# Bluear7878/Remote-Sensing-Vision-Language-Diffusion-Model

Hardware: AMD Instinct MI355X
Metric: 512px x8 SR images/sec @50 steps (higher is better)
Workload: dtype f16 / bf16 MFMA operands as hi + lo pairs and triples, f32 accumulation and f32 residual streams (Stage 1: f16 tensors x f16 weight pairs; Stage 2: rsvld_amd.ops.UNET_POLICY; config.precision) -- the composition inside 1e-3 of the reference's CPU path (config.tolerance)

## Files before the change

include/rsvld_hip.h:

```cpp
#ifndef RSVLD_HIP_H
#define RSVLD_HIP_H

#include <stdint.h>

#ifdef __cplusplus
extern "C" {
#endif

#define RSVLD_OK 0
#define RSVLD_EINVAL (-1)
#define RSVLD_EUNSUPPORTED (-2)
#define RSVLD_ELAUNCH (-3)

#define RSVLD_F16 0
#define RSVLD_BF16 1
#define RSVLD_F32 2
#define RSVLD_SPLIT 3
#define RSVLD_F16W2 4
#define RSVLD_F16Q8 6
#define RSVLD_F16W1 5

#define RSVLD_ACT_NONE 0
#define RSVLD_ACT_SILU 1
#define RSVLD_ACT_GEGLU 2

const char* rsvld_version(void);

typedef struct rsvld_conv_desc {
    const void* x;
    const void* x2;
    const void* w;
    const float* bias;
    const float* rowvec;
    const void* residual;
    void* out;
    int32_t B, H, W, Cin, Cin2, Cout;
    int32_t KH, KW, stride, pad_t, pad_l, Ho, Wo;
    int32_t upsample;
    int32_t dtype;
    int32_t out_f32;
    int32_t act;
    float alpha, beta;
    int32_t rowvec_stride;
    int32_t plan_div;
    int32_t tune;
} rsvld_conv_desc;

#define RSVLD_TUNE_TILE_MASK 7
#define RSVLD_TUNE_STAGES_SHIFT 3
#define RSVLD_TUNE_NO_KSPLIT (1 << 6)
#define RSVLD_TUNE_REG_STAGING (1 << 7)
#define RSVLD_TUNE_HALO_NW4 (1 << 8)
#define RSVLD_TUNE_HALO_NW8 (1 << 9)
#define RSVLD_TUNE_NO_GEMM256 (1 << 10)
#define RSVLD_TUNE_GEMM_ONE_TILE (1 << 12)
#define RSVLD_TUNE_F32_SPLIT (1 << 11)

#define RSVLD_HQ8_SX_LO 14
#define RSVLD_HQ8_SX_HI 2
#define RSVLD_HQ8_SW_HI 6
#define RSVLD_HQ8_SW_LO 18
int rsvld_conv2d_nhwc(const rsvld_conv_desc* d, void* stream);

int rsvld_conv3x3_halo_supported(const rsvld_conv_desc* d);
int rsvld_conv3x3_halo_nhwc(const rsvld_conv_desc* d, const float* norm_scale_shift, int norm_silu,
                            float* out_stats_partials, void* stream);

int64_t rsvld_groupnorm_ws_bytes(int B, int HW, int C, int groups);
int rsvld_groupnorm_nhwc(const void* x, const void* x2, void* y,
                         const float* gamma, const float* beta,
                         const void* mod_scale1p, const void* mod_shift, int mod_stride,
                         int B, int HW, int C1, int C2, int groups, float eps,
                         int silu, int dtype, void* ws, void* stream);
int rsvld_groupnorm_stats(const void* x, const void* x2, float* mean_var,
                          int B, int HW, int C1, int C2, int groups,
                          int dtype, void* ws, void* stream);
int rsvld_groupnorm_apply(const void* x, const void* x2, void* y, const float* mean_var,
                          const float* gamma, const float* beta,
                          const void* mod_scale1p, const void* mod_shift, int mod_stride,
                          int B, int HW, int C1, int C2, int groups, float eps,
                          int silu, int dtype, void* stream);

int rsvld_groupnorm_scale_shift(const void* x, const void* x2, const float* gamma, const float* beta,
                                float* scale_shift, int B, int HW, int C1, int C2, int groups, float eps,
                                int dtype, void* ws, void* stream);

int rsvld_groupnorm_scale_shift_from_partials(const float* part1, int ntiles1, int C1,
                                              const float* part2, int ntiles2, int C2,
                                              const float* gamma, const float* beta, float* scale_shift,
                                              int B, int HW, int groups, float eps, void* stream);

int rsvld_layernorm(const void* x, void* y, const float* gamma, const float* beta,
                    int64_t rows, int C, float eps, int dtype, void* stream);

int rsvld_attention(const void* q, const void* k, const void* v, void* out,
                    int B, int heads, int Nq, int Nk, int D,
                    int64_t q_batch_stride, int64_t q_tok_stride,
                    int64_t k_batch_stride, int64_t k_tok_stride,
                    int64_t v_batch_stride, int64_t v_tok_stride,
                    int64_t o_batch_stride, int64_t o_tok_stride,
                    float scale, int dtype, int plan_div, void* ws, void* stream);
#define RSVLD_ATTN_D64_FOUR_WAVE 1
#define RSVLD_ATTN_D64_PINGPONG 2
#define RSVLD_ATTN_D64_PIPELINED 3
int rsvld_attention_tuned(const void* q, const void* k, const void* v, void* out,
                          int B, int heads, int Nq, int Nk, int D,
                          int64_t q_batch_stride, int64_t q_tok_stride,
                          int64_t k_batch_stride, int64_t k_tok_stride,
                          int64_t v_batch_stride, int64_t v_tok_stride,
                          int64_t o_batch_stride, int64_t o_tok_stride,
                          float scale, int dtype, int plan_div, void* ws, void* stream, int tune);
int64_t rsvld_attention_ws_bytes(int B, int heads, int Nq, int Nk, int D, int plan_div);

int rsvld_linear_small_f32(const float* x, const float* w, const float* b, float* y,
                           int rows, int in_f, int out_f, int act_in, int act_out, void* stream);

int rsvld_sinusoidal_embedding(const float* t, float* out, int rows, int dim, int kind, void* stream);

int rsvld_nchw_f32_to_nhwc(const float* src, void* dst, int B, int C, int H, int W,
                           int Cdst, int c_off, int zero_pad, float scale, int dtype, void* stream);
int rsvld_nhwc_to_nchw_f32(const void* src, float* dst, int B, int C, int H, int W,
                           int Csrc, int c_off, int src_f32, int dtype, void* stream);
int rsvld_axpby(const void* a, const void* b, void* out, int64_t n, float sa, float sb,
                int dtype, void* stream);
int rsvld_geglu(const void* in, void* out, int64_t rows, int C, int dtype, void* stream);

int rsvld_ddpm_step(const float* x, const float* eps_nhwc, const float* noise, float* x_out,
                    int B, int C, int H, int W, int eps_c,
                    float c_recip, float c_recipm1, float coef1, float coef2, float sigma,
                    int clip, void* stream);

int rsvld_denoiser_out(const float* net_out_nhwc, const float* input, float* out,
                       int B, int C, int H, int W, int c_pad, float c_out, float c_skip, void* stream);
int rsvld_lerp_f32(const float* a, const float* b, float* out, int64_t n, float w, void* stream);
int rsvld_axpy_f32(const float* x, const float* y, float* out, int64_t n, float s, void* stream);
int rsvld_euler_step(const float* x_hat, const float* denoised, const float* x_center, float* x_out,
                     int64_t n, float restore_w, float sigma_hat, float dt, void* stream);
int rsvld_tile_blend_accumulate(float* acc, float* cnt, const float* tile, const float* weights,
                                int B, int C, int H, int W, int y0, int x0, int th, int tw, void* stream);
int rsvld_tile_blend_finish(const float* acc, const float* cnt, float* out, int64_t n, void* stream);
int64_t rsvld_absdiff_ws_bytes(int rows, int64_t n_per_row);
int rsvld_absdiff_sums(const void* a, const void* b, float* out, int rows, int64_t n_per_row,
                       int dtype, void* ws, void* stream);

int rsvld_gaussian_sample(const void* moments_nhwc, const float* noise, float* z,
                          int B, int C, int H, int W, int m_c, float scale, int src_f32,
                          int dtype, void* stream);

int rsvld_wavelet_blur(const float* img, float* low, float* high_accum, int planes, int H, int W,
                       int radius, void* stream);
int rsvld_add_f32(const float* a, const float* b, float* out, int64_t n, void* stream);
int rsvld_adain(const float* content, const float* style, float* out, float* ws_stats,
                int planes, int64_t HW, void* stream);

int rsvld_concat_c(const void* a, const void* b, void* out, int64_t rows, int C1, int C2,
                   int dtype, void* stream);

int rsvld_conv2d_nhwc_f32(const rsvld_conv_desc* d, void* stream);
int64_t rsvld_groupnorm_f32_ws_bytes(int B, int HW, int C, int groups);
int rsvld_groupnorm_stats_f32(const float* x, float* mean_var, int B, int HW, int C, int groups, void* ws, void* stream);
int rsvld_groupnorm_apply_f32(const float* x, float* y, const float* mean_var, const float* gamma, const float* beta,
                              const float* mod_scale1p, const float* mod_shift, int mod_stride,
                              int B, int HW, int C, int groups, float eps, int silu, void* stream);
int rsvld_attention_f32(const float* q, const float* k, const float* v, float* out,
                        int B, int heads, int Nq, int Nk, int D,
                        int64_t q_batch_stride, int64_t q_tok_stride,
                        int64_t k_batch_stride, int64_t k_tok_stride,
                        int64_t v_batch_stride, int64_t v_tok_stride,
                        int64_t o_batch_stride, int64_t o_tok_stride,
                        float scale, void* stream);
int rsvld_attention_f32_split(const float* q, const float* k, const float* v, float* out,
                              int B, int heads, int Nq, int Nk, int D,
                              int64_t q_batch_stride, int64_t q_tok_stride,
                              int64_t k_batch_stride, int64_t k_tok_stride,
                              int64_t v_batch_stride, int64_t v_tok_stride,
                              int64_t o_batch_stride, int64_t o_tok_stride,
                              float scale, void* stream);
int rsvld_layernorm_f32(const float* x, float* y, const float* gamma, const float* beta, int64_t rows, int C, float eps,
                        void* stream);
int rsvld_concat_c_f32(const float* a, const float* b, float* out, int64_t rows, int C1, int C2, void* stream);
int rsvld_axpby_f32(const float* a, const float* b, float* out, int64_t n, float sa, float sb, void* stream);
int rsvld_absdiff_sums_f32(const float* a, const float* b, float* out, int rows, int64_t n_per_row, void* stream);
int rsvld_nchw_f32_to_nhwc_f32(const float* src, float* dst, int B, int C, int H, int W,
                               int Cdst, int c_off, int zero_pad, float scale, void* stream);

int rsvld_gemv(const void* w, const void* x, const void* bias, void* y, int N, int K, int dtype, void* stream);
int rsvld_gemv_fused(const void* w, const void* x, const void* bias, const void* norm_w, float norm_eps, const void* residual, int glu,
// ... 44 lines not shown
```

remote-sensing-vision-language-diffusion-model_amd/csrc/attention.hip:

```cpp
#include "rsvld_common.h"
#include <type_traits>
#include <utility>

namespace {

struct AttnArgs {
    const void* q;
    const void* k;
    const void* v;
    void* out;
    int B, heads, Nq, Nk, D;
    int64_t q_bs, q_ts, k_bs, k_ts, v_bs, v_ts, o_bs, o_ts;
    float scale_log2e;
    unsigned long long* dbg;
};

typedef const __attribute__((address_space(1))) void* gptr_t;
typedef __attribute__((address_space(3))) void* lptr_t;

template <typename F, int... I> __device__ __forceinline__ void static_for_impl(F&& f, std::integer_sequence<int, I...>) {
    (f(std::integral_constant<int, I>{}), ...);
}
template <int N, typename F> __device__ __forceinline__ void static_for(F&& f) {
    static_for_impl(f, std::make_integer_sequence<int, N>{});
// ... 253 lines not shown
#define S_NXT snext
#define A5B_STEADY 0
#define dma_kb_s dma_kb
#define dma_k_s dma_k
#define dma_v_s dma_v
#include "attention_d512_body.inc"
#undef dma_kb_s
#undef dma_k_s
#undef dma_v_s
#undef A5B_STEADY
#undef S_CUR
#undef S_NXT
#undef A5B_PAIR
    }
#undef A5B_NOHOOK
#undef A5B_MFMA_NAME
#undef A5B_CHAIN
#undef A5B_STEP4
#if A5B_FINE
#undef A5B_STEPH4
#undef A5B_STEPH
#endif
#undef A5B_STEP
#undef A5B_KREAD

    const float l_tot = l_run + __shfl_xor(l_run, 32);
    if (qrow >= p.Nq) return;
    const float inv = 1.0f / l_tot;
    if (nsplit == 1) {
        T* Ob = (T*)p.out + (int64_t)b * p.o_bs + (int64_t)h * D + (int64_t)qrow * p.o_ts;
#pragma unroll
        for (int dt = 0; dt < 16; ++dt)
#pragma unroll
            for (int g = 0; g < 4; ++g) {
                v4 o;
#pragma unroll
                for (int e = 0; e < 4; ++e) o[e] = (T)(oacc[dt][4 * g + e] * inv);
                *(v4*)(Ob + dt * 32 + 8 * g + 4 * lh) = o;
            }
    } else {
        const int64_t row = ((int64_t)split * gridDim.z + blockIdx.z) * p.Nq + qrow;
        float* Po = part_o + row * D;
#pragma unroll
        for (int dt = 0; dt < 16; ++dt)
#pragma unroll
            for (int g = 0; g < 4; ++g) {
                f32x4 o;
#pragma unroll
                for (int e = 0; e < 4; ++e) o[e] = oacc[dt][4 * g + e] * inv;
                *(f32x4*)(Po + dt * 32 + 8 * g + 4 * lh) = o;
            }
        if (lh == 0) {
            part_ml[row * 2] = m_run;
            part_ml[row * 2 + 1] = l_tot;
        }
    }
}

template <typename T>
__global__ __launch_bounds__(128) void attn_combine_kernel(AttnArgs p, int nsplit, const float* part_o, const float* part_ml) {
    constexpr int D = 512;
    typedef typename Mfma<T>::v4 v4;
    const int qrow = blockIdx.x, bh = blockIdx.y;
    const int b = bh / p.heads, h = bh % p.heads;
    const int64_t nrows = (int64_t)gridDim.y * p.Nq;
    float mmax = -INFINITY;
    for (int i = 0; i < nsplit; ++i) mmax = fmaxf(mmax, part_ml[((int64_t)i * nrows + (int64_t)bh * p.Nq + qrow) * 2]);
    float wsum = 0.f;
    f32x4 acc = {0.f, 0.f, 0.f, 0.f};
    for (int i = 0; i < nsplit; ++i) {
        const int64_t row = (int64_t)i * nrows + (int64_t)bh * p.Nq + qrow;
        const float wi = part_ml[row * 2 + 1] * __builtin_amdgcn_exp2f(part_ml[row * 2] - mmax);
        const f32x4 o = *(const f32x4*)(part_o + row * D + threadIdx.x * 4);
        acc += o * wi;
        wsum += wi;
    }
    const float inv = 1.0f / wsum;
    v4 o;
#pragma unroll
    for (int e = 0; e < 4; ++e) o[e] = (T)(acc[e] * inv);
    *(v4*)((T*)p.out + (int64_t)b * p.o_bs + (int64_t)h * D + (int64_t)qrow * p.o_ts + threadIdx.x * 4) = o;
}

}

namespace {

constexpr int A6B_TILE = 64 * 128;
#ifndef A6B_ABL
#define A6B_ABL 0
#endif
#ifndef A6B_SUMCHK
#define A6B_SUMCHK 1
#endif
#ifndef A6B_KPB8
#define A6B_KPB8 1
#endif
#ifndef A6B_NW16_MIN
#define A6B_NW16_MIN (1 << 30)
#endif
#ifndef A6B_STAMP
#define A6B_STAMP 0
#endif
__device__ __forceinline__ unsigned long long a6b_stamp() {
    unsigned long long t;
    __builtin_amdgcn_sched_barrier(0);
    asm volatile("s_memtime %0\n\ts_waitcnt lgkmcnt(0)" : "=s"(t) :: "memory");
    __builtin_amdgcn_sched_barrier(0);
    return t;
}

#ifndef A6B_OCC4
#define A6B_OCC4 1
#endif
#ifndef A6B_BIAS
#define A6B_BIAS 1
#endif
__device__ __forceinline__ float a6b_add(float a, float b) { return a + b; }

#ifndef A6_STAGE_O
#define A6_STAGE_O 1
#endif
template <typename T>
__device__ __forceinline__ void a6_store_o(char* wbuf, const f32x16 (&oacc)[2], float inv, int q0, int lane, const AttnArgs& p, int b, int h) {
    typedef typename Mfma<T>::v4 v4;
    const int l31 = lane & 31, lh = lane >> 5;
    T* Ob = (T*)p.out + (int64_t)b * p.o_bs + (int64_t)h * 64;
    if (!A6_STAGE_O) {
        if (q0 + l31 >= p.Nq) return;
#pragma unroll
        for (int dt = 0; dt < 2; ++dt)
#pragma unroll
            for (int g = 0; g < 4; ++g) {
                v4 o;
#pragma unroll
                for (int e = 0; e < 4; ++e) o[e] = (T)(oacc[dt][4 * g + e] * inv);
                *(v4*)(Ob + (int64_t)(q0 + l31) * p.o_ts + dt * 32 + 8 * g + 4 * lh) = o;
            }
        return;
    }
#pragma unroll
    for (int dt = 0; dt < 2; ++dt)
#pragma unroll
        for (int g = 0; g < 4; ++g) {
            v4 o;
#pragma unroll
            for (int e = 0; e < 4; ++e) o[e] = (T)(oacc[dt][4 * g + e] * inv);
            *(v4*)(wbuf + l31 * 128 + (((dt * 4 + g) ^ (l31 & 7)) << 4) + lh * 8) = o;
        }
#pragma unroll
    for (int j = 0; j < 4; ++j) {
        const int row = (lane >> 3) + 8 * j, chunk = lane & 7;
        const u32x4 v = *(const u32x4*)(wbuf + row * 128 + ((chunk ^ (row & 7)) << 4));
        if (q0 + row < p.Nq) *(u32x4*)(Ob + (int64_t)(q0 + row) * p.o_ts + chunk * 8) = v;
    }
}

#ifndef A6B_NW8_MIN
#define A6B_NW8_MIN 16384
#endif
template <typename T, int NW>
__global__ __launch_bounds__(64 * NW, A6B_OCC4 ? 4 : 2) void attn_d64b_kernel(AttnArgs p) {
    constexpr int D = 64;
    constexpr int KPB = NW == 8 ? A6B_KPB8 : 1;
    constexpr int NB = 2 * KPB;
    constexpr bool SPLIT = NW == 16;
// ... 373 lines not shown
        return;
    }
    if (qrow >= p.Nq) return;
    T* Ob = (T*)p.out + (int64_t)b * p.o_bs + (int64_t)h * D + (int64_t)qrow * p.o_ts;
#pragma unroll
    for (int dt = 0; dt < 2; ++dt)
#pragma unroll
        for (int g = 0; g < 4; ++g) {
            v4 o;
#pragma unroll
            for (int e = 0; e < 4; ++e) o[e] = (T)(oacc[dt][4 * g + e] * inv);
            *(v4*)(Ob + dt * 32 + 8 * g + 4 * lh) = o;
        }
}

#include "attention_d64c.inc"
#include "attention_d64p.inc"

}

#ifndef A5B_MALL_KEYS
#define A5B_MALL_KEYS 65536
#endif
static void attn512_plan(int B, int heads, int Nq, int Nk, int* nsplit, int* keys_per_split) {
    const int64_t base = (int64_t)((Nq + 127) / 128) * B * heads;
    int ns = 1;
    if (base < 192) {
        ns = (int)((256 + base - 1) / base);
        const int cap = Nk / 256 > 1 ? Nk / 256 : 1;
        if (ns > cap) ns = cap;
        if (ns > 16) ns = 16;
    }
    if (A5B_MALL_KEYS > 0 && Nk > A5B_MALL_KEYS + A5B_MALL_KEYS / 2) {
        const int nm = (Nk + A5B_MALL_KEYS - 1) / A5B_MALL_KEYS;
        if (nm > ns) ns = nm;
    }
    int kps = ((Nk + ns - 1) / ns + 31) / 32 * 32;
    *keys_per_split = kps;
    *nsplit = (Nk + kps - 1) / kps;
}

extern "C" int64_t rsvld_attention_ws_bytes(int B, int heads, int Nq, int Nk, int D, int plan_div) {
    if (D != 512 || B <= 0 || heads <= 0 || Nq <= 0 || Nk <= 0) return 0;
    int ns, kps;
    attn512_plan(plan_div > 1 ? (B + plan_div - 1) / plan_div : B, heads, Nq, Nk, &ns, &kps);
    if (ns == 1) return 0;
    return (int64_t)ns * B * heads * Nq * (512 + 2) * 4;
}

extern "C" int rsvld_attention_tuned(const void* q, const void* k, const void* v, void* out, int B, int heads, int Nq, int Nk,
                                     int D, int64_t q_batch_stride, int64_t q_tok_stride, int64_t k_batch_stride,
                                     int64_t k_tok_stride, int64_t v_batch_stride, int64_t v_tok_stride,
                                     int64_t o_batch_stride, int64_t o_tok_stride, float scale, int dtype, int plan_div,
                                     void* ws, void* stream, int tune) {
    if (!q || !k || !v || !out || B <= 0 || heads <= 0 || Nq <= 0 || Nk <= 0) return RSVLD_EINVAL;
    if (dtype != RSVLD_F16 && dtype != RSVLD_BF16) return RSVLD_EINVAL;
    if ((q_tok_stride | k_tok_stride | v_tok_stride | o_tok_stride | q_batch_stride | k_batch_stride | v_batch_stride |
         o_batch_stride) & 7)
        return RSVLD_EINVAL;
    if (heads > 65535 || B > 65535) return RSVLD_EINVAL;
    AttnArgs a;
    a.q = q; a.k = k; a.v = v; a.out = out;
    a.B = B; a.heads = heads; a.Nq = Nq; a.Nk = Nk; a.D = D;
    a.q_bs = q_batch_stride; a.q_ts = q_tok_stride; a.k_bs = k_batch_stride; a.k_ts = k_tok_stride;
    a.v_bs = v_batch_stride; a.v_ts = v_tok_stride; a.o_bs = o_batch_stride; a.o_ts = o_tok_stride;
    a.scale_log2e = scale * 1.4426950408889634f;
    a.dbg = (A6B_STAMP && D == 64) ? (unsigned long long*)ws : nullptr;
    hipStream_t s = (hipStream_t)stream;
    if (D == 512) {
        int ns, kps;
        attn512_plan(plan_div > 1 ? (B + plan_div - 1) / plan_div : B, heads, Nq, Nk, &ns, &kps);
        if (ns > 1 && ws == nullptr) return RSVLD_EINVAL;
        float* part_o = (float*)ws;
        float* part_ml = ns > 1 ? part_o + (int64_t)ns * B * heads * Nq * 512 : nullptr;
        dim3 grid((unsigned)((Nq + 127) / 128), (unsigned)ns, (unsigned)(B * heads));
        const bool shared = k == v && k_batch_stride == v_batch_stride && k_tok_stride == v_tok_stride;
        auto go = [&](auto kern, auto comb, int smem) -> int {
            static const hipError_t attr = hipFuncSetAttribute((const void*)kern, hipFuncAttributeMaxDynamicSharedMemorySize, smem);
            if (attr != hipSuccess) return RSVLD_ELAUNCH;
            hipLaunchKernelGGL(kern, grid, dim3(256), smem, s, a, kps, part_o, part_ml);
            if (ns > 1) hipLaunchKernelGGL(comb, dim3((unsigned)Nq, (unsigned)(B * heads)), dim3(128), 0, s, a, ns, part_o, part_ml);
            return rsvld_check_launch();
        };
        if (shared)
            return dtype == RSVLD_F16 ? go(attn_d512b_kernel<f16, true>, attn_combine_kernel<f16>, A5B_SMEM_SH)
                                      : go(attn_d512b_kernel<bf16, true>, attn_combine_kernel<bf16>, A5B_SMEM_SH);
        return dtype == RSVLD_F16 ? go(attn_d512b_kernel<f16, false>, attn_combine_kernel<f16>, A5B_SMEM)
                                  : go(attn_d512b_kernel<bf16, false>, attn_combine_kernel<bf16>, A5B_SMEM);
    }
    if (D == 64) {
        const char force = tune == RSVLD_ATTN_D64_FOUR_WAVE ? 'b' : tune == RSVLD_ATTN_D64_PINGPONG ? 'c' : tune == RSVLD_ATTN_D64_PIPELINED ? 'p' : 0;
        if (force == 'p' && Nk > 64 && k_tok_stride < (1 << 23) && v_tok_stride < (1 << 23)) {
            dim3 grid((unsigned)((Nq + 255) / 256), (unsigned)heads, (unsigned)B);
            static const hipError_t a16 = hipFuncSetAttribute((const void*)attn_d64p_kernel<f16>, hipFuncAttributeMaxDynamicSharedMemorySize, A6P_SMEM);
            static const hipError_t abf = hipFuncSetAttribute((const void*)attn_d64p_kernel<bf16>, hipFuncAttributeMaxDynamicSharedMemorySize, A6P_SMEM);
            if (a16 != hipSuccess || abf != hipSuccess) return RSVLD_ELAUNCH;
            if (dtype == RSVLD_F16) hipLaunchKernelGGL((attn_d64p_kernel<f16>), grid, dim3(512), A6P_SMEM, s, a);
            else hipLaunchKernelGGL((attn_d64p_kernel<bf16>), grid, dim3(512), A6P_SMEM, s, a);
            return rsvld_check_launch();
        }
        const int64_t wg_c = (int64_t)((Nq + 511) / 512) * heads * B;
        const bool c_strides_ok = 64 * k_tok_stride * 2 < ((int64_t)1 << 32) && 64 * v_tok_stride * 2 < ((int64_t)1 << 32);
        if (force == 'c' && !c_strides_ok) return RSVLD_EUNSUPPORTED;
        if (c_strides_ok && (a.dbg == nullptr || force == 'c') && force != 'b' && Nk > 64 && ((wg_c >= A6C_MIN_WG && Nk >= A6C_MIN_KEYS) || force == 'c')) {
            dim3 grid((unsigned)((Nq + 511) / 512), (unsigned)heads, (unsigned)B);
            static const hipError_t attr16 = hipFuncSetAttribute((const void*)attn_d64c_kernel<f16>, hipFuncAttributeMaxDynamicSharedMemorySize, A6C_SMEM);
            static const hipError_t attrbf = hipFuncSetAttribute((const void*)attn_d64c_kernel<bf16>, hipFuncAttributeMaxDynamicSharedMemorySize, A6C_SMEM);
            if (attr16 != hipSuccess || attrbf != hipSuccess) return RSVLD_ELAUNCH;
            if (dtype == RSVLD_F16) hipLaunchKernelGGL((attn_d64c_kernel<f16>), grid, dim3(512), A6C_SMEM, s, a);
            else hipLaunchKernelGGL((attn_d64c_kernel<bf16>), grid, dim3(512), A6C_SMEM, s, a);
        } else if (Nq >= A6B_NW16_MIN) {
            dim3 grid((unsigned)((Nq + 511) / 512), (unsigned)heads, (unsigned)B);
            if (dtype == RSVLD_F16) hipLaunchKernelGGL((attn_d64b_kernel<f16, 16>), grid, dim3(1024), 0, s, a);
            else hipLaunchKernelGGL((attn_d64b_kernel<bf16, 16>), grid, dim3(1024), 0, s, a);
        } else if (Nq >= A6B_NW8_MIN) {
            dim3 grid((unsigned)((Nq + 255) / 256), (unsigned)heads, (unsigned)B);
            if (dtype == RSVLD_F16) hipLaunchKernelGGL((attn_d64b_kernel<f16, 8>), grid, dim3(512), 0, s, a);
            else hipLaunchKernelGGL((attn_d64b_kernel<bf16, 8>), grid, dim3(512), 0, s, a);
        } else {
            dim3 grid((unsigned)((Nq + 127) / 128), (unsigned)heads, (unsigned)B);
            if (dtype == RSVLD_F16) hipLaunchKernelGGL((attn_d64b_kernel<f16, 4>), grid, dim3(256), 0, s, a);
            else hipLaunchKernelGGL((attn_d64b_kernel<bf16, 4>), grid, dim3(256), 0, s, a);
        }
        return rsvld_check_launch();
    }
    return RSVLD_EUNSUPPORTED;
}

extern "C" int rsvld_attention(const void* q, const void* k, const void* v, void* out, int B, int heads, int Nq, int Nk,
                               int D, int64_t q_batch_stride, int64_t q_tok_stride, int64_t k_batch_stride,
                               int64_t k_tok_stride, int64_t v_batch_stride, int64_t v_tok_stride,
                               int64_t o_batch_stride, int64_t o_tok_stride, float scale, int dtype, int plan_div,
                               void* ws, void* stream) {
    return rsvld_attention_tuned(q, k, v, out, B, heads, Nq, Nk, D, q_batch_stride, q_tok_stride, k_batch_stride, k_tok_stride,
                                 v_batch_stride, v_tok_stride, o_batch_stride, o_tok_stride, scale, dtype, plan_div, ws, stream, 0);
}
```

remote-sensing-vision-language-diffusion-model_amd/devtools.py:

```python
import os

from . import _lib as L
from . import ops


def tune_from_env(e=None):
    e = os.environ if e is None else e
    t = L.TUNE_TILE.get(e.get("RSVLD_CONV_TILE", ""), 0)
    if e.get("RSVLD_CONV_STAGES"):
        t |= (int(e["RSVLD_CONV_STAGES"]) & 7) << L.TUNE_STAGES_SHIFT
    if e.get("RSVLD_CONV_KSPLIT", "1")[:1] == "0":
        t |= L.TUNE_NO_KSPLIT
    if e.get("RSVLD_CONV_STAGING", "")[:1] == "r":
        t |= L.TUNE_REG_STAGING
    if e.get("RSVLD_HALO_NW"):
        t |= L.TUNE_HALO_NW8 if e["RSVLD_HALO_NW"][:1] == "8" else L.TUNE_HALO_NW4
    if e.get("RSVLD_GEMM256_OFF") is not None:
        t |= L.TUNE_NO_GEMM256
    if e.get("RSVLD_GEMM256_ONE_TILE") is not None:
        t |= L.TUNE_GEMM_ONE_TILE
    return t


def d64_kernel(name):
    ops.set_defaults(d64_kernel={"b": 1, "c": 2, "p": 3}.get(name or "", 0))


def apply_env(e=None):
    e = os.environ if e is None else e
    ops.set_defaults(tune=tune_from_env(e), profile_detail=bool(e.get("RSVLD_PROFILE_DETAIL")))
    d64_kernel(e.get("RSVLD_D64_KERNEL", ""))
    if e.get("RSVLD_HALO_MIN_WGS"):
        ops.set_defaults(halo_min_wgs=int(e["RSVLD_HALO_MIN_WGS"]))
```

remote-sensing-vision-language-diffusion-model_amd/ops.py:

```python
import contextlib
import ctypes as C
import contextvars
import math

import torch

from . import _lib as L

_DT = {torch.float16: L.F16, torch.bfloat16: L.BF16}


def _stream():
    return C.c_void_p(torch.cuda.current_stream().cuda_stream)


def _ptr(t):
    return None if t is None else C.c_void_p(t.data_ptr())


def _need_gpu(*ts):
    for t in ts:
        if t is not None and not t.is_cuda:
            raise L.RsvldError("rsvld_amd ops run on the GPU only (got a CPU tensor); there is no CPU fallback")


def _dt(t):
    try:
        return _DT[t.dtype]
    except KeyError:
        raise L.RsvldError(f"16-bit activation expected, got {t.dtype}")


def pad8(c):
    return (c + 7) // 8 * 8


_HALF = (torch.float16, torch.bfloat16)
_ACT = (torch.float16, torch.bfloat16, torch.float32)


def _bad(fn, name, what):
    raise L.RsvldOperandError(f"{fn}: operand '{name}' {what}")


def _arg(fn, name, t, dtype=None, shape=None, numel=None, layout="contiguous", optional=False):
    if t is None:
        if optional:
            return None
        _bad(fn, name, "is required")
    if not isinstance(t, torch.Tensor):
        _bad(fn, name, f"must be a tensor, got {type(t).__name__}")
    if dtype is not None and t.dtype not in (dtype if isinstance(dtype, tuple) else (dtype,)):
        _bad(fn, name, f"has dtype {t.dtype}, expected {dtype}")
    if shape is not None and (t.dim() != len(shape) or any(s is not None and s != n for s, n in zip(shape, t.shape))):
        _bad(fn, name, f"has shape {tuple(t.shape)}, expected {tuple('*' if s is None else s for s in shape)}")
    if numel is not None and t.numel() != numel:
        _bad(fn, name, f"has {t.numel()} elements, expected {numel}")
    if layout == "contiguous" and not t.is_contiguous():
        _bad(fn, name, f"must be contiguous, got strides {tuple(t.stride())}")
    if layout == "rows" and t.dim():
        vec = max(1, 16 // t.element_size())
        if (t.stride(-1) != 1 and t.shape[-1] > 1) or t.storage_offset() % vec or any(
                s % vec for s, n in zip(t.stride()[:-1], t.shape[:-1]) if n > 1):
            _bad(fn, name, f"must have unit inner stride and 16-byte rows, got strides {tuple(t.stride())} "
                           f"at offset {t.storage_offset()}")
    return t


def _same(fn, name, t, ref, optional=False):
    return _arg(fn, name, t, ref.dtype, shape=tuple(ref.shape), optional=optional)


class LaunchContext:

    __slots__ = ("plan_div", "policy", "tune", "use_halo", "halo_min_wgs", "split_halo_min_wgs", "split_d512_fused_min",
                 "split_attn_s_bytes", "profiler", "profile_detail", "d64_kernel")

    def __init__(self, plan_div=1, policy=None, tune=0, use_halo=True, halo_min_wgs=256, split_halo_min_wgs=64,
                 split_d512_fused_min=2048, split_attn_s_bytes=32 << 30, profiler=None, profile_detail=False, d64_kernel=0):
        object.__setattr__(self, "plan_div", max(1, int(plan_div)))
        for k, v in (("policy", policy), ("tune", int(tune)), ("use_halo", bool(use_halo)), ("halo_min_wgs", int(halo_min_wgs)),
                     ("split_halo_min_wgs", int(split_halo_min_wgs)), ("split_d512_fused_min", int(split_d512_fused_min)),
                     ("split_attn_s_bytes", int(split_attn_s_bytes)), ("profiler", profiler), ("profile_detail", bool(profile_detail)),
                     ("d64_kernel", int(d64_kernel))):
            object.__setattr__(self, k, v)

    def __setattr__(self, k, v):
        raise AttributeError("LaunchContext is immutable: use ops.tuning(...) / ops.plan_units(n) / ops.f32_split(policy) around the calls")

    def replace(self, **changes):
        kw = {k: getattr(self, k) for k in self.__slots__}
        bad = [k for k in changes if k not in kw]
        if bad:
            raise TypeError(f"LaunchContext has no field {bad}")
        kw.update(changes)
        return LaunchContext(**kw)


_CTX = contextvars.ContextVar("rsvld_launch_context", default=LaunchContext())


def context():
    return _CTX.get()


@contextlib.contextmanager
def tuning(**changes):
    token = _CTX.set(_CTX.get().replace(**changes))
    try:
        yield _CTX.get()
    finally:
        _CTX.reset(token)


def set_defaults(**changes):
    _CTX.set(_CTX.get().replace(**changes))


def plan_units(n):
    return tuning(plan_div=max(1, int(n)))


class SplitPolicy:

    __slots__ = ("impl", "f16_inputs", "f16_weights", "q8_convs")
    GROUPS = ("attn", "attn_out", "ff", "qkv", "proj", "conv1", "conv2")
    WEIGHT_GROUPS = ("qkv", "geglu", "attn_out", "ff_out")
    Q8_GROUPS = ("conv1", "conv2")

    def __init__(self, impl="planes", f16_inputs=("attn", "attn_out", "ff", "qkv"), f16_weights=None, q8_convs=None):
        if q8_convs is None:
            q8_convs = (tuple(g for g in self.Q8_GROUPS if g not in f16_inputs)
                        if (impl == "planes" and {"attn", "attn_out", "ff", "qkv"} <= set(f16_inputs)) else ())
        bad = [g for g in q8_convs if g not in self.Q8_GROUPS]
        if bad:
            raise ValueError(f"SplitPolicy.q8_convs {bad}: one of {self.Q8_GROUPS}")
        if set(q8_convs) & set(f16_inputs):
            raise ValueError("SplitPolicy: a convolution's input is either rounded to fp16 (f16_inputs) or kept with e4m3 cross terms (q8_convs)")
        if q8_convs and impl != "planes":
            raise ValueError("SplitPolicy.q8_convs exists in the product path (impl \"planes\") only")
        self.q8_convs = frozenset(q8_convs)
        if f16_weights is None:
            f16_weights = tuple(g for g, i in (("qkv", "qkv"), ("geglu", "ff"), ("attn_out", "attn_out"), ("ff_out", "ff")) if i in f16_inputs and impl == "planes")
        bad = [g for g in f16_weights if g not in self.WEIGHT_GROUPS]
        if bad:
            raise ValueError(f"SplitPolicy.f16_weights {bad}: one of {self.WEIGHT_GROUPS}")
        self.f16_weights = frozenset(f16_weights)
        if impl not in ("planes", "f32"):
            raise ValueError(f"SplitPolicy.impl {impl!r}: planes or f32")
        bad = [g for g in f16_inputs if g not in self.GROUPS]
        if bad:
            raise ValueError(f"SplitPolicy.f16_inputs {bad}: one of {self.GROUPS}")
        self.impl, self.f16_inputs = impl, frozenset(f16_inputs)
        if self.f16_inputs - {"attn"} and "attn" not in self.f16_inputs:
            raise ValueError("SplitPolicy: fp16 layer inputs go with fp16 attention operands (\"attn\")")
        if self.f16_inputs and impl != "planes":
            raise ValueError("SplitPolicy: fp16 layer inputs exist in the product path (impl \"planes\") only")
        need = {"qkv": "qkv", "geglu": "ff", "attn_out": "attn_out", "ff_out": "ff"}
        bad = [g for g in self.f16_weights if need[g] not in self.f16_inputs]
        if bad:
            raise ValueError(f"SplitPolicy.f16_weights {bad}: a layer's weights are rounded to fp16 only where its input is (f16_inputs)")

    def key(self):
        return (self.impl, tuple(sorted(self.f16_inputs)), tuple(sorted(self.f16_weights)), tuple(sorted(self.q8_convs)))

    def describe(self):
        return {"impl": self.impl, "f16_inputs": sorted(self.f16_inputs), "f16_weights": sorted(self.f16_weights), "q8_convs": sorted(self.q8_convs)}
# ... 841 lines not shown
            _ptr(x), _ptr(y), _ptr(stats), _ptr(gamma), _ptr(beta), _ptr(mod_scale1p), _ptr(mod_shift), mod_stride,
            B, H * W, C1, groups, eps, int(silu), _stream()), "rsvld_groupnorm_apply_f32"))
        y._nhwc = True
        return y
    L.check(L.load().rsvld_groupnorm_apply(_ptr(x), _ptr(x2), _ptr(y), _ptr(stats), _ptr(gamma), _ptr(beta), None,
                                           None, 0, B, H * W, C1, C2, groups, eps, int(silu), _dt(x), _stream()),
            "rsvld_groupnorm_apply")
    return y


def layer_norm(x, gamma, beta, eps=1e-5, planes=False, group=None):
    _arg("layer_norm", "x", x, _ACT)
    if x.dim() < 1 or x.numel() == 0:
        _bad("layer_norm", "x", f"needs rows of channels, got shape {tuple(x.shape)}")
    Cc = x.shape[-1]
    _arg("layer_norm", "gamma", gamma, torch.float32, shape=(Cc,), optional=True)
    _arg("layer_norm", "beta", beta, torch.float32, shape=(Cc,), optional=True)
    _need_gpu(x, gamma, beta)
    rows = x.numel() // Cc
    if x.dtype == torch.float32 and _split_fast():
        if not x.is_contiguous():
            raise L.RsvldError("layer_norm (split): contiguous rows expected")
        f16 = planes and f16_group(group)
        if f16:
            y = torch.empty(x.shape, device=x.device, dtype=torch.float16)
        elif planes:
            y = torch.empty(tuple(x.shape[:-1]) + (2, Cc), device=x.device, dtype=torch.bfloat16)
        else:
            y = torch.empty_like(x)
        _launch("layernorm_split", 0.0, (6.0 if f16 else 8.0) * x.numel(), lambda: L.check(L.load().rsvld_layernorm_split(
            _ptr(x), _ptr(y), _ptr(gamma), _ptr(beta), rows, Cc, eps, 2 if f16 else int(not planes), _stream()), "rsvld_layernorm_split"))
        return y if f16 else (Planes(y) if planes else y)
    y = torch.empty_like(x)
    if x.dtype == torch.float32:
        if not x.is_contiguous():
            raise L.RsvldError("layer_norm (fp32): contiguous rows expected")
        _launch("layernorm_f32", 0.0, 8.0 * x.numel(), lambda: L.check(L.load().rsvld_layernorm_f32(
            _ptr(x), _ptr(y), _ptr(gamma), _ptr(beta), rows, Cc, eps, _stream()), "rsvld_layernorm_f32"))
        return y
    L.check(L.load().rsvld_layernorm(_ptr(x), _ptr(y), _ptr(gamma), _ptr(beta), rows, Cc, eps, _dt(x), _stream()),
            "rsvld_layernorm")
    return y


def attention(q, k, v, heads, scale=None):
    split = any(isinstance(t, Planes) for t in (q, k, v)) or (q.dtype == torch.float32 and _split_fast())
    for name, t in (("q", q), ("k", k), ("v", v)):
        if isinstance(t, Planes):
            _arg("attention", name, t.t, torch.bfloat16, shape=(None, None, 2, None), layout=None)
        else:
            _arg("attention", name, t, (torch.float32, torch.float16) if split else (_ACT if t is q else q.dtype), shape=(None,) * 3,
                 layout="rows")
    if heads <= 0 or q.shape[2] % heads:
        _bad("attention", "q", f"has {q.shape[2]} channels, not a multiple of heads = {heads}")
    for name, t in (("k", k), ("v", v)):
        if tuple(t.shape) != (q.shape[0], k.shape[1], q.shape[2]):
            _bad("attention", name, f"has shape {tuple(t.shape)}, expected [B, Nk, H*D] = {(q.shape[0], k.shape[1], q.shape[2])}")
    if split:
        return _attention_split(q, k, v, heads, scale)
    _need_gpu(q, k, v)
    B, Nq, HD = q.shape
    Nk = k.shape[1]
    D = HD // heads
    if scale is None:
        scale = 1.0 / math.sqrt(D)
    for t in (q, k, v):
        if t.stride(2) != 1:
            raise L.RsvldError("attention: last dim must be contiguous")
    out = torch.empty((B, Nq, HD), device=q.device, dtype=q.dtype)
    lib = L.load()
    flops = 4.0 * B * heads * Nq * Nk * D
    nbytes = (q.shape[0] * Nq * HD * 2 + 2 * B * Nk * HD) * q.element_size()
    if q.dtype == torch.float32:
        if k.dtype != torch.float32 or v.dtype != torch.float32:
            raise L.RsvldError("attention (fp32): q, k, v must all be fp32")
        fn = lib.rsvld_attention_f32_split if _policy() is not None else lib.rsvld_attention_f32
        _launch(f"attention_f32{'_split' if _policy() is not None else ''}_d{D}", flops, nbytes, lambda: L.check(
            fn(_ptr(q), _ptr(k), _ptr(v), _ptr(out), B, heads, Nq, Nk, D,
               q.stride(0), q.stride(1), k.stride(0), k.stride(1), v.stride(0), v.stride(1),
               out.stride(0), out.stride(1), scale, _stream()), "rsvld_attention_f32"))
        return out
    ws_bytes = lib.rsvld_attention_ws_bytes(B, heads, Nq, Nk, D, _CTX.get().plan_div)
    ws = torch.empty(ws_bytes, device=q.device, dtype=torch.uint8) if ws_bytes > 0 else None
    tune = _CTX.get().d64_kernel
    _launch(f"attention_d{D}" + ("_cross" if (D == 64 and Nk != Nq) else ""), flops, nbytes, lambda: L.check(
        lib.rsvld_attention_tuned(_ptr(q), _ptr(k), _ptr(v), _ptr(out), B, heads, Nq, Nk, D,
                                  q.stride(0), q.stride(1), k.stride(0), k.stride(1), v.stride(0), v.stride(1),
                                  out.stride(0), out.stride(1), scale, _dt(q), _CTX.get().plan_div, _ptr(ws), _stream(), tune),
        "rsvld_attention"))
    if _split_fast() and not f16_group("attn_out"):
        return _f16_to_planes(out)
    return out


def _split_gemm(xt, w3, out, M, K, N, out_f32, name):
    d = L.ConvDesc(x=xt.data_ptr(), x2=None, w=w3.data_ptr(), bias=None, rowvec=None, residual=None, out=out.data_ptr(),
                   B=1, H=1, W=M, Cin=K, Cin2=0, Cout=N, KH=1, KW=1, stride=1, pad_t=0, pad_l=0, Ho=1, Wo=M, upsample=0,
                   dtype=L.SPLIT, out_f32=int(out_f32), act=L.ACT_NONE, alpha=1.0, beta=1.0, rowvec_stride=0, plan_div=1, tune=_CTX.get().tune)
    _launch(name, 2.0 * M * K * N, 4.0 * M * K + 6.0 * N * K + 4.0 * M * N,
            lambda: L.check(L.load().rsvld_conv2d_nhwc(C.byref(d), _stream()), "rsvld_conv2d_nhwc"))


def _planes_to_f16(x):
    if not isinstance(x, Planes):
        return x.to(torch.float16)
    t = x.t
    B, N, _, C = t.shape
    if t.stride(3) != 1 or t.stride(0) != N * t.stride(1):
        t = t.contiguous()
    out = torch.empty((B, N, C), device=t.device, dtype=torch.float16)
    _launch("planes_to_f16", 0.0, 6.0 * B * N * C, lambda: L.check(L.load().rsvld_planes_to_f16(
        _ptr(t), t.stride(1), t.stride(2), _ptr(out), C, B * N, C, _stream()), "rsvld_planes_to_f16"))
    return out


def _f16_to_planes(x):
    C = x.shape[-1]
    t = torch.empty(tuple(x.shape[:-1]) + (2, C), device=x.device, dtype=torch.bfloat16)
    _launch("f16_to_planes", 0.0, 6.0 * x.numel(), lambda: L.check(L.load().rsvld_f16_to_planes(
        _ptr(x), C, _ptr(t), x.numel() // C, C, _stream()), "rsvld_f16_to_planes"))
    return Planes(t)


def _attention_split(q, k, v, heads, scale):
    if f16_group("attn") and q.shape[-1] % 8 == 0:
        shared = k is v
        q16, k16 = _planes_to_f16(q), _planes_to_f16(k)
        v16 = k16 if shared else _planes_to_f16(v)
        return attention(q16, k16, v16, heads, scale)
    return _attention_split_kernels(q, k, v, heads, scale)


def _attention_split_kernels(q, k, v, heads, scale):
    shared = k is v
    def prep(t):
        if isinstance(t, Planes):
            return t
        return to_planes(t.contiguous())
    q = prep(q)
    k = prep(k)
    v = k if shared else prep(v)
    _need_gpu(q.t, k.t, v.t)
    B, Nq, HD = q.shape
    Nk = k.shape[1]
    D = HD // heads
    if scale is None:
        scale = 1.0 / math.sqrt(D)
    lib = L.load()
    out = torch.empty((B, Nq, 2, HD), device=q.t.device, dtype=torch.bfloat16)
    flops = 4.0 * B * heads * Nq * Nk * D
    if D == 64:
        for t in (q.t, k.t, v.t):
            if t.stride(3) != 1:
                raise L.RsvldError("attention (split): last dim must be contiguous")
        nbytes = 4.0 * (2 * B * Nq * HD + 2 * B * Nk * HD)
        _launch("attention_split_d64" + ("_cross" if Nk != Nq else ""), flops, nbytes, lambda: L.check(lib.rsvld_attention_split_d64(
            _ptr(q.t), _ptr(k.t), _ptr(v.t), _ptr(out), B, heads, Nq, Nk,
            q.t.stride(0), q.t.stride(1), q.t.stride(2), k.t.stride(0), k.t.stride(1), k.t.stride(2),
            v.t.stride(0), v.t.stride(1), v.t.stride(2), out.stride(0), out.stride(1), out.stride(2), scale, 0, _stream()),
            "rsvld_attention_split_d64"))
        return Planes(out)
    if D == 512 and heads == 1 and shared and Nq >= _CTX.get().split_d512_fused_min:
        nbytes = 4.0 * (2 * B * Nq * HD + B * Nk * HD)
        _launch("attention_split_d512", flops, nbytes, lambda: L.check(lib.rsvld_attention_split_d512_shared(
            _ptr(q.t), _ptr(k.t), _ptr(out), B, Nq, Nk, q.t.stride(0), q.t.stride(1), q.t.stride(2),
            k.t.stride(0), k.t.stride(1), k.t.stride(2), out.stride(0), out.stride(1), out.stride(2), scale, 0, _stream()),
            "rsvld_attention_split_d512_shared"))
# ... 343 lines not shown
```

Measured before the change: 0.01342.

## Add D-split d512 shared-KV attention kernel with cross-wave P exchange

Adds a new D=512 attention kernel for the shared K=V case and makes it the default. Each of the four waves computes the score tile for its own 32 query rows, then shares its probability fragments and rescale factors through LDS. Each wave then accumulates PV for a 128-wide slice of the head dimension across all 128 rows. The K chain is hand-scheduled with inline asm and uses a 4-deep LDS DMA ring and paired score accumulators to overlap softmax with the next tile's QK MFMAs. The aim is to reuse the V fragments across rows and cut per-wave accumulator and V-read cost, in exchange for an extra __syncthreads per tile and a lot of complex asm. The old row kernel stays reachable through a new tuning knob.

```diff
diff --git a/include/rsvld_hip.h b/include/rsvld_hip.h
--- a/include/rsvld_hip.h
+++ b/include/rsvld_hip.h
@@ -103,6 +103,8 @@
 #define RSVLD_ATTN_D64_FOUR_WAVE 1
 #define RSVLD_ATTN_D64_PINGPONG 2
 #define RSVLD_ATTN_D64_PIPELINED 3
+#define RSVLD_ATTN_D512_ROWS 4
+#define RSVLD_ATTN_D512_DSPLIT 5
 int rsvld_attention_tuned(const void* q, const void* k, const void* v, void* out,
                           int B, int heads, int Nq, int Nk, int D,
                           int64_t q_batch_stride, int64_t q_tok_stride,
diff --git a/remote-sensing-vision-language-diffusion-model_amd/csrc/attention.hip b/remote-sensing-vision-language-diffusion-model_amd/csrc/attention.hip
--- a/remote-sensing-vision-language-diffusion-model_amd/csrc/attention.hip
+++ b/remote-sensing-vision-language-diffusion-model_amd/csrc/attention.hip
@@ -359,6 +359,8 @@
     *(v4*)((T*)p.out + (int64_t)b * p.o_bs + (int64_t)h * D + (int64_t)qrow * p.o_ts + threadIdx.x * 4) = o;
 }
 
+#include "attention_d512d.inc"
+
 }
 
 namespace {
@@ -898,6 +900,9 @@
             if (ns > 1) hipLaunchKernelGGL(comb, dim3((unsigned)Nq, (unsigned)(B * heads)), dim3(128), 0, s, a, ns, part_o, part_ml);
             return rsvld_check_launch();
         };
+        if (shared && tune != RSVLD_ATTN_D512_ROWS)
+            return dtype == RSVLD_F16 ? go(attn_d512d_kernel<f16>, attn_combine_kernel<f16>, A5D_SMEM)
+                                      : go(attn_d512d_kernel<bf16>, attn_combine_kernel<bf16>, A5D_SMEM);
         if (shared)
             return dtype == RSVLD_F16 ? go(attn_d512b_kernel<f16, true>, attn_combine_kernel<f16>, A5B_SMEM_SH)
                                       : go(attn_d512b_kernel<bf16, true>, attn_combine_kernel<bf16>, A5B_SMEM_SH);
diff --git a/remote-sensing-vision-language-diffusion-model_amd/csrc/attention_d512d.inc b/remote-sensing-vision-language-diffusion-model_amd/csrc/attention_d512d.inc
--- /dev/null
+++ b/remote-sensing-vision-language-diffusion-model_amd/csrc/attention_d512d.inc
@@ -0,0 +1,212 @@
+constexpr int A5D_P_OFF = 4 * A5B_TILE;
+constexpr int A5D_PBUF = 4 * 2 * 64 * 16;
+constexpr int A5D_A_OFF = A5D_P_OFF + 2 * A5D_PBUF;
+constexpr int A5D_L_OFF = A5D_A_OFF + 2 * 512;
+constexpr int A5D_SMEM = A5D_L_OFF + 512;
+
+template <typename T>
+__global__ __launch_bounds__(256) void attn_d512d_kernel(AttnArgs p, int keys_per_split, float* part_o, float* part_ml) {
+    constexpr int D = 512;
+    typedef typename Mfma<T>::v8 v8;
+    typedef typename Mfma<T>::v4 v4;
+    extern __shared__ __attribute__((aligned(16))) char smem[];
+
+    const int tid = threadIdx.x, lane = tid & 63, w = tid >> 6;
+    const int l31 = lane & 31, lh = lane >> 5;
+    const int q0 = blockIdx.x * 128 + w * 32;
+    const int split = blockIdx.y, nsplit = gridDim.y;
+    const int b = blockIdx.z / p.heads, h = blockIdx.z % p.heads;
+    const int k_begin = split * keys_per_split;
+    const int k_end = min(p.Nk, k_begin + keys_per_split);
+    const int nt = (k_end - k_begin + 31) >> 5;
+    const T* Qb = (const T*)p.q + (int64_t)b * p.q_bs + (int64_t)h * D;
+    const T* Xb = (const T*)p.k + (int64_t)b * p.k_bs + (int64_t)h * D;
+
+    const int wu = __builtin_amdgcn_readfirstlane(w);
+    const uint32_t lds0 = (uint32_t)(uintptr_t)(lptr_t)smem;
+    auto dma_one = [&](const char* base, uint32_t voff, uint32_t dst) {
+        asm volatile("s_mov_b32 m0, %1\n\ts_nop 0\n\tglobal_load_lds_dwordx4 %0, %2" : : "v"(voff), "s"(dst), "s"(base) : "memory", "m0");
+    };
+    const int64_t x_rowb = p.k_ts * (int64_t)sizeof(T);
+    const uint32_t lane16 = (uint32_t)lane << 4;
+    const char* x_tile0 = (const char*)(Xb + (int64_t)(k_begin + wu * 8) * p.k_ts);
+    auto dma_x = [&](int t, int i) {
+        const int r = wu * 8 + i;
+        const uint32_t dst = lds0 + (t & 3) * A5B_TILE + r * 1024;
+        if (k_begin + t * 32 + 32 <= p.Nk) {
+            dma_one(x_tile0 + (int64_t)(t * 32 + i) * x_rowb, lane16 ^ (uint32_t)(a5b_f(r & 15) << 4), dst);
+        } else {
+            const int key = min(k_begin + t * 32 + r, p.Nk - 1);
+            dma_one((const char*)(Xb + (int64_t)key * p.k_ts), lane16 ^ (uint32_t)(a5b_f(r & 15) << 4), dst);
+        }
+    };
+    auto dma_x_fast = [&](int t, int i) {
+        const int r = wu * 8 + i;
+        dma_one(x_tile0 + (int64_t)(t * 32 + i) * x_rowb, lane16 ^ (uint32_t)(a5b_f(r & 15) << 4), lds0 + (t & 3) * A5B_TILE + r * 1024);
+    };
+#pragma unroll
+    for (int i = 0; i < 8; ++i) dma_x(0, i);
+    if (nt > 1) {
+#pragma unroll
+        for (int i = 0; i < 8; ++i) dma_x(1, i);
+    }
+    if (nt > 2) {
+#pragma unroll
+        for (int i = 0; i < 8; ++i) dma_x(2, i);
+    }
+
+    const int qrow = q0 + l31;
+    v8 qf[32];
+#pragma unroll
+    for (int ks = 0; ks < 32; ++ks) {
+        u32x4 v = {0u, 0u, 0u, 0u};
+        if (qrow < p.Nq) v = *(const u32x4*)(Qb + (int64_t)qrow * p.q_ts + ks * 16 + lh * 8);
+        qf[ks] = __builtin_bit_cast(v8, v);
+    }
+    f32x16 oacc[4][4];
+#pragma unroll
+    for (int dt = 0; dt < 4; ++dt)
+#pragma unroll
+        for (int j = 0; j < 4; ++j)
+#pragma unroll
+            for (int r = 0; r < 16; ++r) oacc[dt][j][r] = 0.f;
+    float m_run = -INFINITY, l_run = 0.f;
+
+    const uint32_t kb = l31 * 1024 + ((lh ^ a5b_f(l31 & 15)) << 4);
+    int vbase[4];
+    {
+        const int qq = (lane >> 2) & 3, pp = lane & 3, g1 = (lane >> 4) & 1;
+#pragma unroll
+        for (int f = 0; f < 4; ++f) vbase[f] = (4 * lh + qq) * 1024 + ((f ^ qq) << 6) + (((2 * g1 + (pp >> 1)) ^ lh) << 4) + ((pp & 1) << 3) + wu * 256;
+    }
+    auto vread = [&](int buf, int f, int s2) {
+        const int off = buf * A5B_TILE + vbase[f] + (16 * s2) * 1024;
+        const s16x4 lo = __builtin_amdgcn_ds_read_tr16_b64_v4i16((__attribute__((address_space(3))) s16x4*)(smem + off));
+        const s16x4 hi = __builtin_amdgcn_ds_read_tr16_b64_v4i16((__attribute__((address_space(3))) s16x4*)(smem + ((off ^ 32) + 8 * 1024)));
+        typedef short s16x8 __attribute__((__vector_size__(8 * sizeof(short))));
+        return __builtin_bit_cast(v8, (s16x8)__builtin_shufflevector(lo, hi, 0, 1, 2, 3, 4, 5, 6, 7));
+    };
+    const int p_own = A5D_P_OFF + wu * 2048 + lane * 16, a_own = A5D_A_OFF + l31 * 16 + wu * 4;
+    int p_oth[3], a_oth[3];
+#pragma unroll
+    for (int j = 1; j < 4; ++j) {
+        p_oth[j - 1] = A5D_P_OFF + ((wu + j) & 3) * 2048 + lane * 16;
+        a_oth[j - 1] = A5D_A_OFF + l31 * 16 + ((wu + j) & 3) * 4;
+    }
+
+    asm volatile("s_waitcnt vmcnt(0)" ::: "memory");
+    __syncthreads();
+
+    constexpr int KD = 6;
+    uint32_t ka[8];
+    v8 kfr[KD];
+#define A5D_KREAD(slot, ks) \
+    asm volatile("ds_read_b128 %0, %1 offset:%2" : "=v"(kfr[slot]) : "v"(ka[(ks) & 7]), "i"(((ks) >> 3) * 256))
+#define A5D_STEP(NAME, SACC, ks)                                                                                        \
+    asm volatile("s_waitcnt lgkmcnt(%3)\n\t" NAME " %0, %1, %2, %0"                                                      \
+                 : "+v"(SACC)                                                                                           \
+                 : "v"(kfr[(ks) % KD]), "v"(qf[ks]), "i"(KD - 1 < 31 - (ks) ? KD - 1 : 31 - (ks)));                      \
+    if constexpr ((ks) + KD < 32) A5D_KREAD((ks) % KD, (ks) + KD)
+#define A5D_STEP4(NAME, SACC, k) \
+    A5D_STEP(NAME, SACC, k); A5D_STEP(NAME, SACC, (k) + 1); A5D_STEP(NAME, SACC, (k) + 2); A5D_STEP(NAME, SACC, (k) + 3)
+#define A5D_CHAIN(NAME, SACC, KBUF, HOOK)                                                                               \
+    _Pragma("unroll") for (int c = 0; c < 8; ++c) ka[c] = lds0 + (((KBUF) * A5B_TILE + kb) ^ (c << 5));         \
+    A5D_KREAD(0, 0); A5D_KREAD(1, 1); A5D_KREAD(2, 2); A5D_KREAD(3, 3); A5D_KREAD(4, 4); A5D_KREAD(5, 5);               \
+    asm volatile("s_waitcnt lgkmcnt(%3)\n\t" NAME " %0, %1, %2, 0" : "=&v"(SACC) : "v"(kfr[0]), "v"(qf[0]), "i"(KD - 1)); \
+    A5D_KREAD(0, KD);                                                                                                   \
+    A5D_STEP(NAME, SACC, 1); A5D_STEP(NAME, SACC, 2); A5D_STEP(NAME, SACC, 3); HOOK(0);                                 \
+    A5D_STEP4(NAME, SACC, 4); HOOK(1); A5D_STEP4(NAME, SACC, 8); HOOK(2); A5D_STEP4(NAME, SACC, 12); HOOK(3);           \
+    A5D_STEP4(NAME, SACC, 16); HOOK(4); A5D_STEP4(NAME, SACC, 20); HOOK(5); A5D_STEP4(NAME, SACC, 24); HOOK(6);         \
+    A5D_STEP4(NAME, SACC, 28); HOOK(7)
+#define A5D_NOHOOK(i)
+
+    f32x16 sacc;
+    if constexpr (__is_same(T, f16)) {
+        A5D_CHAIN("v_mfma_f32_32x32x16_f16", sacc, 0, A5D_NOHOOK);
+    } else {
+        A5D_CHAIN("v_mfma_f32_32x32x16_bf16", sacc, 0, A5D_NOHOOK);
+    }
+    asm volatile("s_nop 15\n\ts_nop 3" : "+v"(sacc));
+
+    int t = 0;
+    f32x16 sacc2;
+#define A5D_STEADY 1
+#define A5D_PAIR 1
+    for (; t + 5 < nt;) {
+        {
+#define S_CUR sacc
+#define S_NXT sacc2
+#include "attention_d512d_body.inc"
+#undef S_CUR
+#undef S_NXT
+        }
+        ++t;
+        {
+#define S_CUR sacc2
+#define S_NXT sacc
+#include "attention_d512d_body.inc"
+#undef S_CUR
+#undef S_NXT
+        }
+        ++t;
+    }
+#undef A5D_PAIR
+#undef A5D_STEADY
+    for (; t < nt; ++t) {
+#define A5D_PAIR 0
+#define A5D_STEADY 0
+#define S_CUR sacc
+#define S_NXT snext
+#include "attention_d512d_body.inc"
+#undef S_NXT
+#undef S_CUR
+#undef A5D_STEADY
+#undef A5D_PAIR
+    }
+#undef A5D_NOHOOK
+#undef A5D_CHAIN
+#undef A5D_STEP4
+#undef A5D_STEP
+#undef A5D_KREAD
+
+    const float l_tot = l_run + __shfl_xor(l_run, 32);
+    *(float*)(smem + A5D_L_OFF + l31 * 16 + wu * 4) = l_tot;
+    __syncthreads();
+    float inv[4];
+    inv[0] = 1.0f / l_tot;
+#pragma unroll
+    for (int j = 1; j < 4; ++j) inv[j] = 1.0f / *(const float*)(smem + A5D_L_OFF + l31 * 16 + ((wu + j) & 3) * 4);
+#pragma unroll
+    for (int j = 0; j < 4; ++j) {
+        const int qr = blockIdx.x * 128 + ((wu + j) & 3) * 32 + l31;
+        if (qr >= p.Nq) continue;
+        if (nsplit == 1) {
+            T* Ob = (T*)p.out + (int64_t)b * p.o_bs + (int64_t)h * D + (int64_t)qr * p.o_ts + wu * 128;
+#pragma unroll
+            for (int dt = 0; dt < 4; ++dt)
+#pragma unroll
+                for (int g = 0; g < 4; ++g) {
+                    v4 o;
+#pragma unroll
+                    for (int e = 0; e < 4; ++e) o[e] = (T)(oacc[dt][j][4 * g + e] * inv[j]);
+                    *(v4*)(Ob + dt * 32 + 8 * g + 4 * lh) = o;
+                }
+        } else {
+            const int64_t row = ((int64_t)split * gridDim.z + blockIdx.z) * p.Nq + qr;
+            float* Po = part_o + row * D + wu * 128;
+#pragma unroll
+            for (int dt = 0; dt < 4; ++dt)
+#pragma unroll
+                for (int g = 0; g < 4; ++g) {
+                    f32x4 o;
+#pragma unroll
+                    for (int e = 0; e < 4; ++e) o[e] = oacc[dt][j][4 * g + e] * inv[j];
+                    *(f32x4*)(Po + dt * 32 + 8 * g + 4 * lh) = o;
+                }
+            if (j == 0 && lh == 0) {
+                part_ml[row * 2] = m_run;
+                part_ml[row * 2 + 1] = l_tot;
+            }
+        }
+    }
+}
diff --git a/remote-sensing-vision-language-diffusion-model_amd/csrc/attention_d512d_body.inc b/remote-sensing-vision-language-diffusion-model_amd/csrc/attention_d512d_body.inc
--- /dev/null
+++ b/remote-sensing-vision-language-diffusion-model_amd/csrc/attention_d512d_body.inc
@@ -0,0 +1,126 @@
+        const bool more = A5D_STEADY ? true : t + 1 < nt;
+        const int b_pv = t & 3, pb = (t & 1) * A5D_PBUF, ab = (t & 1) * 512;
+
+        float mx = -INFINITY, alpha = 1.0f, rs = 0.f;
+        bool need = false;
+        v8 pf[2];
+        auto sm = [&](int part) {
+            if (part == 0) {
+                if (!A5D_STEADY && k_begin + (t + 1) * 32 > k_end) {
+#pragma unroll
+                    for (int r = 0; r < 16; ++r) {
+                        const int kv = k_begin + t * 32 + (r & 3) + 8 * (r >> 2) + 4 * lh;
+                        if (kv >= k_end) S_CUR[r] = -INFINITY;
+                    }
+                }
+#pragma unroll
+                for (int r = 0; r < 16; ++r) mx = fmaxf(mx, S_CUR[r]);
+                asm volatile("" : "+v"(S_CUR), "+v"(mx));
+            } else if (part == 1) {
+                mx = a5b_halfwave_max(mx) * p.scale_log2e;
+                need = mx > m_run + A5_DEFER_LOG2;
+                if (need) {
+                    alpha = __builtin_amdgcn_exp2f(m_run - mx);
+                    m_run = mx;
+                }
+                asm volatile("" : "+v"(alpha), "+v"(m_run));
+            } else if (part >= 2 && part <= 5) {
+                const int r0 = 4 * (part - 2);
+#pragma unroll
+                for (int r = r0; r < r0 + 4; ++r) {
+                    S_CUR[r] = __builtin_amdgcn_exp2f(__builtin_fmaf(S_CUR[r], p.scale_log2e, -m_run));
+                    rs += S_CUR[r];
+                }
+                asm volatile("" : "+v"(S_CUR[r0]), "+v"(S_CUR[r0 + 1]), "+v"(S_CUR[r0 + 2]), "+v"(S_CUR[r0 + 3]), "+v"(rs));
+            } else if (part == 6) {
+                l_run = l_run * alpha + rs;
+#pragma unroll
+                for (int s2 = 0; s2 < 2; ++s2)
+#pragma unroll
+                    for (int j = 0; j < 8; ++j) pf[s2][j] = (T)S_CUR[8 * s2 + j];
+                asm volatile("" : "+v"(pf[0]), "+v"(pf[1]), "+v"(l_run));
+            }
+        };
+#if !A5D_PAIR
+        f32x16 snext;
+#endif
+        if (more) {
+#define A5D_HOOK(i) \
+    sm(i);          \
+    __builtin_amdgcn_sched_barrier(0)
+            if constexpr (__is_same(T, f16)) {
+                A5D_CHAIN("v_mfma_f32_32x32x16_f16", S_NXT, ((t + 1) & 3), A5D_HOOK);
+            } else {
+                A5D_CHAIN("v_mfma_f32_32x32x16_bf16", S_NXT, ((t + 1) & 3), A5D_HOOK);
+            }
+#undef A5D_HOOK
+        } else {
+#pragma unroll
+            for (int i = 0; i < 7; ++i) sm(i);
+        }
+
+        *(v8*)(smem + pb + p_own) = pf[0];
+        *(v8*)(smem + pb + p_own + 1024) = pf[1];
+        *(float*)(smem + ab + a_own) = alpha;
+        v8 vfr[2][4];
+#pragma unroll
+        for (int s2 = 0; s2 < 2; ++s2)
+#pragma unroll
+            for (int f = 0; f < 4; ++f) vfr[s2][f] = vread(b_pv, f, s2);
+        asm volatile("s_waitcnt vmcnt(0)" ::: "memory");
+        __syncthreads();
+
+        v8 pfo[2][3];
+        float al[3];
+#pragma unroll
+        for (int s2 = 0; s2 < 2; ++s2)
+#pragma unroll
+            for (int j = 0; j < 3; ++j) pfo[s2][j] = *(const v8*)(smem + pb + p_oth[j] + 1024 * s2);
+#pragma unroll
+        for (int j = 0; j < 3; ++j) al[j] = *(const float*)(smem + ab + a_oth[j]);
+
+#define A5D_RESCALE(J, A)                                                                                                  \
+    _Pragma("unroll") for (int dt = 0; dt < 4; ++dt)                                                                       \
+    _Pragma("unroll") for (int r = 0; r < 16; ++r) {                                                                       \
+        float x = oacc[dt][J][r], tmp;                                                                                     \
+        asm volatile("v_accvgpr_read_b32 %1, %0\n\tv_mul_f32 %1, %1, %2\n\ts_nop 0\n\tv_accvgpr_write_b32 %0, %1\n\ts_nop 1" \
+                     : "+a"(x), "=&v"(tmp)                                                                                 \
+                     : "v"(A));                                                                                            \
+        oacc[dt][J][r] = x;                                                                                                \
+    }
+        if (__builtin_expect(__any(need), 0)) {
+            asm volatile("s_nop 15\n\ts_nop 3" ::: "memory");
+            A5D_RESCALE(0, alpha)
+        }
+        __builtin_amdgcn_sched_barrier(0);
+#pragma unroll
+        for (int s2 = 0; s2 < 2; ++s2)
+#pragma unroll
+            for (int f = 0; f < 4; ++f) {
+                oacc[f][0] = Mfma<T>::mma(vfr[s2][f], pf[s2], oacc[f][0]);
+                __builtin_amdgcn_sched_barrier(0);
+            }
+        if (__builtin_expect(__any(al[0] != 1.0f || al[1] != 1.0f || al[2] != 1.0f), 0)) {
+            asm volatile("s_nop 15\n\ts_nop 3" ::: "memory");
+            A5D_RESCALE(1, al[0])
+            A5D_RESCALE(2, al[1])
+            A5D_RESCALE(3, al[2])
+        }
+#undef A5D_RESCALE
+        __builtin_amdgcn_sched_barrier(0);
+#pragma unroll
+        for (int n = 0; n < 24; ++n) {
+            const int s2 = n / 12, f = (n / 3) & 3, j = n % 3;
+            oacc[f][j + 1] = Mfma<T>::mma(vfr[s2][f], pfo[s2][j], oacc[f][j + 1]);
+            if (n % 3 == 2) {
+                if (A5D_STEADY) {
+                    dma_x_fast(t + 3, n / 3);
+                } else if (t + 3 < nt) {
+                    dma_x(t + 3, n / 3);
+                }
+            }
+            __builtin_amdgcn_sched_barrier(0);
+        }
+#if !A5D_PAIR
+        if (more) S_CUR = S_NXT;
+#endif
diff --git a/remote-sensing-vision-language-diffusion-model_amd/devtools.py b/remote-sensing-vision-language-diffusion-model_amd/devtools.py
--- a/remote-sensing-vision-language-diffusion-model_amd/devtools.py
+++ b/remote-sensing-vision-language-diffusion-model_amd/devtools.py
@@ -26,9 +26,14 @@
     ops.set_defaults(d64_kernel={"b": 1, "c": 2, "p": 3}.get(name or "", 0))
 
 
+def d512_kernel(name):
+    ops.set_defaults(d512_kernel={"rows": 4, "dsplit": 5}.get(name or "", 0))
+
+
 def apply_env(e=None):
     e = os.environ if e is None else e
     ops.set_defaults(tune=tune_from_env(e), profile_detail=bool(e.get("RSVLD_PROFILE_DETAIL")))
     d64_kernel(e.get("RSVLD_D64_KERNEL", ""))
+    d512_kernel(e.get("RSVLD_D512_KERNEL", ""))
     if e.get("RSVLD_HALO_MIN_WGS"):
         ops.set_defaults(halo_min_wgs=int(e["RSVLD_HALO_MIN_WGS"]))
diff --git a/remote-sensing-vision-language-diffusion-model_amd/ops.py b/remote-sensing-vision-language-diffusion-model_amd/ops.py
--- a/remote-sensing-vision-language-diffusion-model_amd/ops.py
+++ b/remote-sensing-vision-language-diffusion-model_amd/ops.py
@@ -74,15 +74,16 @@
 class LaunchContext:
 
     __slots__ = ("plan_div", "policy", "tune", "use_halo", "halo_min_wgs", "split_halo_min_wgs", "split_d512_fused_min",
-                 "split_attn_s_bytes", "profiler", "profile_detail", "d64_kernel")
+                 "split_attn_s_bytes", "profiler", "profile_detail", "d64_kernel", "d512_kernel")
 
     def __init__(self, plan_div=1, policy=None, tune=0, use_halo=True, halo_min_wgs=256, split_halo_min_wgs=64,
-                 split_d512_fused_min=2048, split_attn_s_bytes=32 << 30, profiler=None, profile_detail=False, d64_kernel=0):
+                 split_d512_fused_min=2048, split_attn_s_bytes=32 << 30, profiler=None, profile_detail=False, d64_kernel=0,
+                 d512_kernel=0):
         object.__setattr__(self, "plan_div", max(1, int(plan_div)))
         for k, v in (("policy", policy), ("tune", int(tune)), ("use_halo", bool(use_halo)), ("halo_min_wgs", int(halo_min_wgs)),
                      ("split_halo_min_wgs", int(split_halo_min_wgs)), ("split_d512_fused_min", int(split_d512_fused_min)),
                      ("split_attn_s_bytes", int(split_attn_s_bytes)), ("profiler", profiler), ("profile_detail", bool(profile_detail)),
-                     ("d64_kernel", int(d64_kernel))):
+                     ("d64_kernel", int(d64_kernel)), ("d512_kernel", int(d512_kernel))):
             object.__setattr__(self, k, v)
 
     def __setattr__(self, k, v):
@@ -1090,7 +1091,7 @@
         return out
     ws_bytes = lib.rsvld_attention_ws_bytes(B, heads, Nq, Nk, D, _CTX.get().plan_div)
     ws = torch.empty(ws_bytes, device=q.device, dtype=torch.uint8) if ws_bytes > 0 else None
-    tune = _CTX.get().d64_kernel
+    tune = _CTX.get().d64_kernel if D == 64 else _CTX.get().d512_kernel
     _launch(f"attention_d{D}" + ("_cross" if (D == 64 and Nk != Nq) else ""), flops, nbytes, lambda: L.check(
         lib.rsvld_attention_tuned(_ptr(q), _ptr(k), _ptr(v), _ptr(out), B, heads, Nq, Nk, D,
                                   q.stride(0), q.stride(1), k.stride(0), k.stride(1), v.stride(0), v.stride(1),
```

New measurement: 0.01368 (median of 6 runs). +1.9%, better.
